# JeffOwOSun/ntm-tracker

Measured on AMD Instinct MI355X. Metric: frames/sec (whole node) VGG16+NTM(128x20) seq_len=20, higher is better.
Workload: dtype f32

## Files before the change

include/ntmtrack.h:

```cpp
#ifndef NTMTRACK_H_
#define NTMTRACK_H_

#include <stddef.h>
#include <stdint.h>

#ifdef __cplusplus
extern "C" {
#endif

#define NTK_OK               0
#define NTK_ERR_BAD_SHAPE   -1
#define NTK_ERR_BAD_PTR     -2
#define NTK_ERR_UNSUPPORTED -3
#define NTK_ERR_HIP         -4

int ntk_version(void);
const char* ntk_last_error(void);


int ntk_vgg_packed_k(int cin);
int ntk_vgg_pack_weights(const float* w_hwio, float* w_packed, int cin, int cout, void* stream);

int ntk_vgg_conv3x3_relu_f32(const float* in, const float* w_packed, const float* bias,
                             float* out, int frames, int H, int W, int cin, int cout,
// ... 4 lines not shown
                              int frames, int H, int W, int cin, int cout, int fuse_pool, int out_f32,
                              void* stream);
size_t ntk_vgg_bf16p_packed_elems(int cin, int cout);
int ntk_vgg_bf16p_supported(int H, int W, int cin, int cout, int fuse_pool);
int ntk_vgg_pack_weights_bf16p(const float* w_hwio, void* w_packed_bf16, int cin, int cout, int H, int W, void* stream);
int ntk_vgg_conv3x3_relu_bf16p(const void* in_bf16, const void* w_packed_bf16p, const float* bias, void* out,
                               int frames, int H, int W, int cin, int cout, int fuse_pool, int out_f32, void* stream);
int ntk_vgg_conv3x3_relu_f32_to_bf16(const float* in, const float* w_packed, const float* bias, void* out_bf16,
                                     int frames, int H, int W, int cin, int cout, void* stream);

size_t ntk_vgg_split3_packed_elems(int cin, int cout);
int ntk_vgg_split3_supported(int H, int W, int cin, int cout, int fuse_pool);
int ntk_vgg_pack_weights_split3(const float* w_hwio, void* w_packed, int cin, int cout, int H, int W, void* stream);
int ntk_vgg_conv3x3_relu_split3(const void* in_split, const void* w_packed, const float* bias, void* out,
                                int frames, int H, int W, int cin, int cout, int fuse_pool, int in_f32, int out_f32, void* stream);

size_t ntk_vgg_wino_packed_floats(int cin, int cout);
int ntk_vgg_wino_supported(int frames, int H, int W, int cin, int cout);
int ntk_vgg_pack_weights_wino(const float* w_hwio, float* u_packed, int cin, int cout, void* stream);
int ntk_vgg_conv3x3_relu_wino_f32(const float* in, const float* u_packed, const float* bias, float* out,
                                  int frames, int H, int W, int cin, int cout, int fuse_pool, void* stream);

size_t ntk_vgg_wino43_packed_floats(int cin, int cout);
int ntk_vgg_wino43_supported(int frames, int H, int W, int cin, int cout);
int ntk_vgg_wino43_blocked_supported(int frames, int H, int W, int cin, int cout);
int ntk_vgg_pack_weights_wino43(const float* w_hwio, float* u_packed, int cin, int cout, void* stream);
int ntk_vgg_conv3x3_relu_wino43_f32(const float* in, const float* u_packed, const float* bias, float* out,
                                    int frames, int H, int W, int cin, int cout, int fuse_pool, void* stream);
int ntk_vgg_conv3x3_relu_wino43_window_f32(const float* in, const float* u_packed, const float* bias, float* out,
                                           int frames, int H, int W, int cin, int cout, int fuse_pool,
// ... 426 lines not shown
```

ntm-tracker_amd/_lib.py:

```python
import ctypes
import os

import torch

_HERE = os.path.dirname(os.path.abspath(__file__))
LIB_PATH = os.environ.get("NTK_LIB_PATH") or os.path.join(_HERE, "libntmtrack_hip.so")

_lib = None


class NtkError(RuntimeError):
    pass


def _sig(lib):
    c_int, c_void_p, c_size_t = ctypes.c_int, ctypes.c_void_p, ctypes.c_size_t
    P = c_void_p
    sigs = {
        "ntk_version": (c_int, []),
        "ntk_last_error": (ctypes.c_char_p, []),
        "ntk_vgg_packed_k": (c_int, [c_int]),
        "ntk_vgg_pack_weights": (c_int, [P, P, c_int, c_int, P]),
        "ntk_vgg_conv3x3_relu_f32": (c_int, [P, P, P, P, c_int, c_int, c_int, c_int, c_int, c_int, P]),
        "ntk_vgg_pack_weights_bf16": (c_int, [P, P, c_int, c_int, P]),
        "ntk_vgg_conv3x3_relu_bf16": (c_int, [P, P, P, P] + [c_int] * 7 + [P]),
        "ntk_vgg_conv3x3_relu_f32_to_bf16": (c_int, [P, P, P, P] + [c_int] * 5 + [P]),
        "ntk_vgg_bf16p_packed_elems": (c_size_t, [c_int, c_int]),
        "ntk_vgg_bf16p_supported": (c_int, [c_int] * 5),
        "ntk_vgg_pack_weights_bf16p": (c_int, [P, P] + [c_int] * 4 + [P]),
        "ntk_vgg_conv3x3_relu_bf16p": (c_int, [P, P, P, P] + [c_int] * 7 + [P]),
        "ntk_vgg_split3_packed_elems": (c_size_t, [c_int, c_int]),
        "ntk_vgg_split3_supported": (c_int, [c_int] * 5),
        "ntk_vgg_pack_weights_split3": (c_int, [P, P] + [c_int] * 4 + [P]),
        "ntk_vgg_conv3x3_relu_split3": (c_int, [P, P, P, P] + [c_int] * 8 + [P]),
        "ntk_gemm_nt_f32": (c_int, [P, c_int, P, c_int, P, P, c_int, c_int, c_int, c_int, P]),
        "ntk_gemm_tn_workspace_bytes": (c_size_t, [c_int, c_int, c_int]),
        "ntk_gemm_tn_f32": (c_int, [P, c_int, P, c_int, P, c_int, c_int, c_int, c_int, c_int, c_int, P, P]),
        "ntk_ntm_padded_dims": (c_int, [c_int] * 7 + [ctypes.POINTER(c_int)] * 5),
        "ntk_ntm_seq_fwd": (c_int, [c_int] * 10 + [P] * 23 + [P]),
        "ntk_transpose_pad": (c_int, [P, c_int, P, c_int, c_int, c_int, P]),
        "ntk_ntm_seq_bwd": (c_int, [c_int] * 10 + [P, c_int, P, c_int] + [P] * 21 + [P]),
        "ntk_ntm_seq_deep_supported": (c_int, [c_int] * 9),
        "ntk_ntm_seq_plan": (c_int, [c_int] * 11 + [ctypes.POINTER(c_int)] * 4),
        "ntk_ntm_seq_deep_plan": (c_int, [c_int] * 10 + [ctypes.POINTER(c_int)] * 4),
        "ntk_ntm_seq_deep_packed_floats": (c_int, [c_int] * 5 + [ctypes.POINTER(c_size_t)] * 3),
        "ntk_ntm_seq_deep_pack": (c_int, [c_int] * 5 + [P] * 6 + [P]),
        "ntk_ntm_seq_fwd_deep": (c_int, [c_int] * 12 + [P] * 29 + [P]),
        "ntk_ntm_seq_bwd_deep": (c_int, [c_int] * 11 + [P, P, c_int] + [P] * 24 + [P]),
        "ntk_dnc_padded_dims": (c_int, [c_int] * 6 + [ctypes.POINTER(c_int)] * 8),
# ... 133 lines not shown
```

ntm-tracker_amd/csrc/conv_bf16p.hip:

```cpp
#include "conv_tiles.h"

#ifndef BF16P_ABL
#define BF16P_ABL 0
#endif

namespace {

typedef __bf16 pbf16x8 __attribute__((ext_vector_type(8)));
typedef __bf16 pbf16x4 __attribute__((ext_vector_type(4)));


struct Bf16pArgs {
    const __bf16* in; const __bf16* wq; const float* bias; void* out;
    int frames, H, W, Cin, Cout;
    int bxN, byN;
    int NQ, NS;
    int nCB;
};

typedef int pv4i __attribute__((ext_vector_type(4)));
__device__ __forceinline__ void p_dma16(pv4i rs, unsigned lds_addr, int voff, int soff) {
    unsigned keep;
    asm volatile("s_mov_b32 %0, m0\n\ts_mov_b32 m0, %1\n\ts_nop 0\n\tbuffer_load_dwordx4 %2, %3, %4 offen lds\n\ts_mov_b32 m0, %0"
                 : "=&s"(keep) : "s"(lds_addr), "v"(voff), "s"(rs), "s"(soff) : "memory");
}
__device__ __forceinline__ pv4i p_rsrc(const void* base, unsigned bytes) {
    const unsigned long long p = (unsigned long long)base;
    return pv4i{(int)(unsigned)p, (int)(unsigned)(p >> 32), (int)bytes, 0x00020000};
}

__device__ __forceinline__ pbf16x8 p_as_bf16x8(const f32x4& v) {
    union { f32x4 f; pbf16x8 b; } u;
// ... 67 lines not shown
        const int e = idx & 7;
        size_t r = idx >> 3;
        const int slot = (int)(r & 3); r >>= 2;
        const int n = (int)(r % BN); r /= BN;
        const int tap = (int)(r % 9); r /= 9;
        const int chunk = (int)(r % NC);
        const int cb = (int)(r / NC);
        const int piece = slot ^ p_sw<4>(n);
        const int c = chunk * 16 + (piece & 1) * 8 + e;
        const float v = w[((size_t)tap * Cin + c) * Cout + (size_t)cb * BN + n] * wscale;
        const _Float16 hi = (_Float16)v;
        wq[idx] = (piece & 2) ? (_Float16)(v - (float)hi) : hi;
    }
}

template <int BN, int TW, int TH, int NSUB, int KC, bool POOL, bool OUTF32, int NW = 8, bool X3 = false, bool INF32 = false>
__global__ __launch_bounds__(64 * NW) __attribute__((amdgpu_waves_per_eu(2, 2))) void conv3x3_relu_bf16p_kernel(Bf16pArgs a) {
    static_assert(!INF32 || (X3 && NW == 4), "fp32 input: split form on four waves (the eight-wave form has no registers for the staging)");
    constexpr int PNT = 2 * NW;
    constexpr bool ROWS = (TW & (TW - 1)) != 0;
    static_assert(!X3 || KC == 32, "split form: 16 real channels = one 32-channel chunk");
    static_assert(!ROWS || (!POOL && NSUB == 1 && (TW - 1 + 32 * PNT - 1) / TW + 1 <= TH - 1 && NW == 8), "runs of rows: no row pairs; TH = the patch's image rows");
    static_assert(NW == 8 || (NW == 4 && BN == 64), "four-wave workgroups take 64 columns");
    constexpr int PW = ROWS ? 32 : TW + 2, PH = TH + 2, SPX = PW * PH, NPX = NSUB * SPX;
    static_assert(!ROWS || TW + 2 <= 32, "runs of rows: the patch row pitch is 32");
    constexpr int PIXB = KC * 2, PIECES = KC / 8, PPP = 1024 / PIXB;
    constexpr int NPA = (NPX + PPP - 1) / PPP;
    constexpr int ABYTES = NPA * 1024;
    constexpr int STAPS = KC == 16 ? 9 : 3, SPC = 9 / STAPS;
    constexpr int SBYTES = STAPS * BN * PIXB, NPB = SBYTES / 1024;
    constexpr int NPAW = (NPA + NW - 1) / NW;
    constexpr int TM = BN == 128 ? 4 : 2;
    constexpr int TPS = (TW * TH) / 32;
    constexpr int K16 = KC / 16;
    static_assert(ROWS || NSUB * TW * TH == 32 * PNT, "512 (256) output pixels per workgroup");
    constexpr int TRB = POOL ? 0 : NW * TM * 32 * 144;
    constexpr int LDSB = (2 * ABYTES + 2 * SBYTES) > TRB ? (2 * ABYTES + 2 * SBYTES) : TRB;
    static_assert(LDSB + 1024 <= (NW == 8 ? 160 : 80) * 1024, "LDS");
    __shared__ __attribute__((aligned(1024))) unsigned char s_mem[LDSB];
    __shared__ int s_sbf[NSUB], s_sby[NSUB], s_sbx[NSUB];
    __shared__ __attribute__((aligned(16))) float s_bias[BN + 4];

    const int tid = threadIdx.x, lane = tid & 63;
    const int wave = __builtin_amdgcn_readfirstlane(tid >> 6);
    int cb, sp;
    conv_tile_wg(blockIdx.x, a.nCB, cb, sp);
    if (sp >= a.NS) return;
    const int H = a.H, W = a.W, Cin = a.Cin, Cout = a.Cout;
    const int rP0 = sp * (32 * PNT), rg0 = ROWS ? rP0 / TW : 0, rf0 = ROWS ? rg0 / H : 0, ry0 = ROWS ? rg0 - rf0 * H : 0;
    if (tid < BN) s_bias[tid] = a.bias[cb * BN + tid];
    if (X3 && tid == BN) s_bias[BN] = *reinterpret_cast<const float*>(a.wq + (size_t)9 * a.Cin * a.Cout);
    if constexpr (!ROWS) conv_tile_subblocks<NSUB>(s_sbf, s_sby, s_sbx, tid, sp, a.NQ, a.bxN, a.byN, TH, TW, 0, 0);
    __syncthreads();

    auto a_sw = [](int p) { return ROWS ? ((((p & 31) + 28 * (p >> 5)) >> 2) & 3) : p_sw<PIECES>(p); };
    const int f0 = ROWS ? rf0 : ((sp * NSUB) / a.bxN) / a.byN;
    const size_t in_left = (size_t)(a.frames - f0) * H * W * Cin * sizeof(__bf16);
    const unsigned in_bytes = (unsigned)(in_left < 0x7ffffff0ull ? in_left : 0x7ffffff0ull);
    const __bf16* pin = a.in + (size_t)f0 * H * W * Cin;
    unsigned aoff[NPAW];
#pragma unroll
    for (int i = 0; i < NPAW; ++i) {
        const int pa = wave + NW * i;
        const int lp = pa * PPP + lane / PIECES, slot = lane % PIECES;
        aoff[i] = 0x80000000u;
        if (pa < NPA && lp < NPX) {
            const int q = lp / SPX, rem = lp - q * SPX;
            const int py = rem / PW, px = rem - py * PW;
// ... 27 lines not shown
                const int y = s_sby[q] - 1 + py, x = s_sbx[q] - 1 + px;
                if (fq >= 0 && y >= 0 && y < H && x >= 0 && x < W)
                    foff[i] = (unsigned)(((((size_t)(fq - f0) * H + y) * W + x) * Cin) * sizeof(__bf16) + qd * 16);
            }
        }
    }
    auto f32_rsrc = [&](int chunk) {
        return __builtin_amdgcn_make_buffer_rsrc(const_cast<__bf16*>(pin + (size_t)chunk * KC), 0, (int)(in_bytes - (unsigned)chunk * PIXB), 0x00020000);
    };
    auto f32_put = [&](const f32x4& v, int dst) {
        ph16x4 h, l;
        f32x4 c;
#pragma unroll
        for (int e = 0; e < 4; ++e) c[e] = __builtin_amdgcn_fmed3f(v[e], -S3_MAX, S3_MAX);
        s3_split4(c, h, l);
        *reinterpret_cast<ph16x4*>(s_mem + dst) = h;
        *reinterpret_cast<ph16x4*>(s_mem + (dst ^ 32)) = l;
    };
    const unsigned lds0 = (unsigned)(size_t)(__attribute__((address_space(3))) void*)s_mem;
    auto dma_patch = [&](int chunk, int buf, int i0, int i1) {
        const pv4i rs = p_rsrc(pin + (size_t)chunk * KC, in_bytes - (unsigned)chunk * PIXB);
#pragma unroll
        for (int i = 0; i < NPAW; ++i) {
            if (i >= i0 && i < i1 && wave + NW * i < NPA)
                p_dma16(rs, lds0 + buf * ABYTES + (wave + NW * i) * 1024, (int)aoff[i], 0);
        }
    };
    auto dma_patch1 = [&](int chunk, int buf, auto ic) {
        constexpr int i = decltype(ic)::value;
        const pv4i rs = p_rsrc(pin + (size_t)chunk * KC, in_bytes - (unsigned)chunk * PIXB);
// ... 59 lines not shown
    for (int tm = 0; tm < TM; ++tm)
#pragma unroll
        for (int nt = 0; nt < 2; ++nt)
#pragma unroll
            for (int r = 0; r < 16; ++r) acc[tm][nt][r] = 0.f;
    const int wa0 = 2 * ABYTES + (wn * 64 + mcol) * PIXB + ((kh ^ p_sw<PIECES>(mcol)) << 4);

    if constexpr (INF32) {
        const __amdgpu_buffer_rsrc_t rs = f32_rsrc(0);
        f32x4 v[NIT];
#pragma unroll
        for (int i = 0; i < NIT; ++i) v[i] = __builtin_bit_cast(f32x4, __builtin_amdgcn_raw_buffer_load_b128(rs, (int)foff[i], 0, 0));
#pragma unroll
        for (int i = 0; i < NIT; ++i)
            if (fdst[i] >= 0) f32_put(v[i], fdst[i]);
    } else {
        dma_patch(0, 0, 0, NPAW);
    }
    dma_weights(0, 0);
    asm volatile("s_waitcnt vmcnt(0)" ::: "memory");
    __syncthreads();

    auto stage_body = [&](int chunk, auto part_c) {
        constexpr int part = decltype(part_c)::value;
        const int s = SPC * chunk + part;
        const int abuf = chunk & 1, bbuf = s & 1;
        constexpr int NDW = (NPB + NW - 1) / NW;
        constexpr int NDP = INF32 ? 0 : (NPAW + SPC - 1) / SPC;
        const bool more_w = !(BF16P_ABL & 1) && s + 1 < NSTG, more_p = !(BF16P_ABL & 1) && chunk + 1 < NC;
        auto dma_slot = [&](auto kc) {
            constexpr int k = decltype(kc)::value;
            if constexpr (k < NDW) { if (more_w) dma_weights1(s + 1, bbuf ^ 1, k); }
            else if constexpr (k < NDW + NDP && part * NDP + (k - NDW) < NPAW) {
                if (more_p) dma_patch1(chunk + 1, abuf ^ 1, ntk_ic<part * NDP + (k - NDW)>{});
            }
        };
        const int wa = wa0 + bbuf * SBYTES;
        f32x4 fst[NITS];
        if constexpr (INF32) {
            const __amdgpu_buffer_rsrc_t rs = f32_rsrc(more_p ? chunk + 1 : chunk);
#pragma unroll
            for (int j = 0; j < NITS; ++j)
                if (part * NITS + j < NIT) fst[j] = __builtin_bit_cast(f32x4, __builtin_amdgcn_raw_buffer_load_b128(rs, (int)foff[part * NITS + j], 0, 0));
        }
        if constexpr (X3) {
            f32x4 wh[2][2], wl[2], xh[TM], xl[TM];
            auto ld_w = [&](auto dc, auto kc, f32x4 (&w)[2]) {
                constexpr int dxi = decltype(dc)::value, k16 = decltype(kc)::value;
#pragma unroll
                for (int nt = 0; nt < 2; ++nt)
                    w[nt] = *reinterpret_cast<const f32x4*>(s_mem + ((wa ^ (k16 << 5)) + (dxi * BN + nt * 32) * PIXB));
// ... 9 lines not shown
                for (int tm = 0; tm < TM; ++tm)
#pragma unroll
                    for (int nt = 0; nt < 2; ++nt)
                        acc[tm][nt] = __builtin_amdgcn_mfma_f32_32x32x16_f16(p_as_f16x8(w[nt]), p_as_f16x8(x[tm]), acc[tm][nt], 0, 0, 0);
            };
            using I0 = ntk_ic<0>;
            using I1 = ntk_ic<1>;
            constexpr int NSS = STAPS * 3;
            static_assert(NDW + NDP <= NSS, "one DMA per sub-step");
            auto tapstep = [&](auto dc) {
                constexpr int dxi = decltype(dc)::value;
                if constexpr (!(BF16P_ABL & 4)) ld_w(dc, I1{}, wl);
                __builtin_amdgcn_sched_barrier(0);
                mm(wh[dxi & 1], xh);
                dma_slot(ntk_ic<3 * dxi>{});
                __builtin_amdgcn_sched_barrier(0);
                if constexpr (!(BF16P_ABL & 4)) ld_x(dc, I1{}, xl);
                __builtin_amdgcn_sched_barrier(0);
                mm(wl, xh);
                dma_slot(ntk_ic<3 * dxi + 1>{});
                __builtin_amdgcn_sched_barrier(0);
                if constexpr (dxi + 1 < STAPS && !(BF16P_ABL & 4)) {
                    ld_w(ntk_ic<dxi + 1>{}, I0{}, wh[(dxi + 1) & 1]);
                    ld_x(ntk_ic<dxi + 1>{}, I0{}, xh);
                }
                __builtin_amdgcn_sched_barrier(0);
                mm(wh[dxi & 1], xl);
                dma_slot(ntk_ic<3 * dxi + 2>{});
                __builtin_amdgcn_sched_barrier(0);
            };
            ld_w(I0{}, I0{}, wh[0]);
            ld_x(I0{}, I0{}, xh);
            if constexpr ((BF16P_ABL & 4) != 0) {
#pragma unroll
                for (int nt = 0; nt < 2; ++nt) { wh[1][nt] = wh[0][nt]; wl[nt] = wh[0][nt]; }
#pragma unroll
                for (int tm = 0; tm < TM; ++tm) xl[tm] = xh[tm];
            }
            ntk_static_for<0, STAPS>(tapstep);
            if constexpr (INF32) {
                if (more_p) {
#pragma unroll
                    for (int j = 0; j < NITS; ++j)
// ... 145 lines not shown
            for (int j = 0; j < TM * 4; ++j) {
                const int tmr = j >> 2, mr = 8 * (j & 3) + (lane >> 3), piece = lane & 7;
                const f32x4 v = *reinterpret_cast<const f32x4*>(tr + (tmr * 32 + mr) * RB + piece * 16);
                const int opx = __builtin_amdgcn_ds_bpermute(mr << 2, opix[tmr]);
                if ((BF16P_ABL & 32) ? (opx >= 0 && v[0] == 12345.f) : (opx >= 0)) {
                    const size_t op = (size_t)opx * Cout + cb * BN + wn * 64;
                    if constexpr (OUTF32) *reinterpret_cast<f32x4*>(reinterpret_cast<float*>(a.out) + op + ps * 32 + piece * 4) = v;
                    else if constexpr (X3) *reinterpret_cast<f32x4*>(reinterpret_cast<__bf16*>(a.out) + 2 * (op + ps * 32) + piece * 8) = v;
                    else *reinterpret_cast<f32x4*>(reinterpret_cast<__bf16*>(a.out) + op + piece * 8) = v;
                }
            }
        }
    }
}

template <int BN, int KC, int NW, bool X3 = false, bool INF32 = false>
int bf16p_launch(const Bf16pArgs& a0, int H, int W, int pool, int out_f32, hipStream_t st) {
    Bf16pArgs a = a0;
    if constexpr (X3 && !INF32) {
        if (W == 28) {
            if (pool || NW != 8 || H < 20) return NTK_ERR_UNSUPPORTED;
            a.bxN = 1; a.byN = 1;
            const long long NQ = (long long)a.frames * H * W, NS = (NQ + 511) / 512;
            a.NQ = 0; a.NS = (int)NS; a.nCB = a.Cout / BN;
            const unsigned grid = (unsigned)conv_tile_grid(NS, a.nCB);
            if constexpr (NW == 8) {
                if (out_f32) conv3x3_relu_bf16p_kernel<BN, 28, 21, 1, 32, false, true, 8, true><<<grid, 512, 0, st>>>(a);
                else conv3x3_relu_bf16p_kernel<BN, 28, 21, 1, 32, false, false, 8, true><<<grid, 512, 0, st>>>(a);
            }
            return NTK_OK;
        }
    }
    int shape;
    if (NW == 8) shape = (W % 32 == 0 && H % 16 == 0) ? 0 : ((W % 16 == 0 && H % 16 == 0) ? 1 : ((W % 8 == 0 && H % 8 == 0) ? 2 : 3));
    else shape = (W % 32 == 0 && H % 8 == 0) ? 0 : ((W % 16 == 0 && H % 16 == 0) ? 1 : ((W % 8 == 0 && H % 8 == 0) ? 2 : 3));
    static const int TWs[4] = {32, 16, 8, 4}, THs8[4] = {16, 16, 8, 4}, THs4[4] = {8, 16, 8, 4}, NSUB8[4] = {1, 2, 8, 32}, NSUB4[4] = {1, 1, 4, 16};
    const int TWv = TWs[shape], THv = NW == 8 ? THs8[shape] : THs4[shape], NSUBv = NW == 8 ? NSUB8[shape] : NSUB4[shape];
    a.bxN = W / TWv;
    a.byN = H / THv;
    const long long NQ = (long long)a.frames * a.bxN * a.byN;
    const long long NS = (NQ + NSUBv - 1) / NSUBv;
    a.NQ = (int)NQ; a.NS = (int)NS; a.nCB = a.Cout / BN;
    const unsigned grid = (unsigned)conv_tile_grid(NS, a.nCB);
#define BF16P_GO(TW_, TH_, NSUB_)                                                                                             \
    do {                                                                                                                      \
        if (pool) {                                                                                                           \
            if (out_f32) conv3x3_relu_bf16p_kernel<BN, TW_, TH_, NSUB_, KC, true, true, NW, X3, INF32><<<grid, 64 * NW, 0, st>>>(a);     \
            else conv3x3_relu_bf16p_kernel<BN, TW_, TH_, NSUB_, KC, true, false, NW, X3, INF32><<<grid, 64 * NW, 0, st>>>(a);            \
        } else {                                                                                                              \
            if (out_f32) conv3x3_relu_bf16p_kernel<BN, TW_, TH_, NSUB_, KC, false, true, NW, X3, INF32><<<grid, 64 * NW, 0, st>>>(a);    \
            else conv3x3_relu_bf16p_kernel<BN, TW_, TH_, NSUB_, KC, false, false, NW, X3, INF32><<<grid, 64 * NW, 0, st>>>(a);           \
        }                                                                                                                     \
    } while (0)
    if constexpr (KC == 32 && NW == 8) {
        if (shape == 0) BF16P_GO(32, 16, 1);
        else if (shape == 1) BF16P_GO(16, 16, 2);
        else if (shape == 2) BF16P_GO(8, 8, 8);
        else return NTK_ERR_UNSUPPORTED;
    } else if constexpr (KC == 32) {
        if (shape == 0) BF16P_GO(32, 8, 1);
        else if (shape == 1) BF16P_GO(16, 16, 1);
        else if (shape == 2) BF16P_GO(8, 8, 4);
        else return NTK_ERR_UNSUPPORTED;
    } else {
        if (shape == 3 && !pool && NW == 8) {
            if (out_f32) conv3x3_relu_bf16p_kernel<BN, 4, 4, 32, KC, false, true><<<grid, 512, 0, st>>>(a);
// ... 114 lines not shown
    a.in = reinterpret_cast<const __bf16*>(in_split); a.wq = reinterpret_cast<const __bf16*>(w_packed); a.bias = bias; a.out = out;
    a.frames = frames; a.H = H; a.W = W; a.Cin = 2 * cin; a.Cout = cout;
    a.bxN = a.byN = a.NQ = a.NS = a.nCB = 0;
    int rc;
    hipStream_t st = (hipStream_t)stream;
    NTK_REQUIRE(!in_f32 || nw == 4, NTK_ERR_UNSUPPORTED,
                "ntk_vgg_conv3x3_relu_split3: an fp32 input map is read by the four-wave form only (cin <= 64, cout = 64, H and W multiples of 8)");
    if (nw == 4 && in_f32) rc = bf16p_launch<64, 32, 4, true, true>(a, H, W, fuse_pool, out_f32, st);
    else if (nw == 4) rc = bf16p_launch<64, 32, 4, true>(a, H, W, fuse_pool, out_f32, st);
    else if (bn == 128) rc = bf16p_launch<128, 32, 8, true>(a, H, W, fuse_pool, out_f32, st);
    else rc = bf16p_launch<64, 32, 8, true>(a, H, W, fuse_pool, out_f32, st);
    NTK_REQUIRE(rc == NTK_OK, rc, "ntk_vgg_conv3x3_relu_split3: no instantiation for this shape");
    NTK_CHECK_LAUNCH("ntk_vgg_conv3x3_relu_split3");
    return NTK_OK;
}
```

ntm-tracker_amd/vgg.py:

```python
import math
import os
from collections import namedtuple

import torch

from . import _lib

VGG_LAYERS = [
    ("conv1_1", 3, 64, False), ("conv1_2", 64, 64, True),
    ("conv2_1", 64, 128, False), ("conv2_2", 128, 128, True),
    ("conv3_1", 128, 256, False), ("conv3_2", 256, 256, False), ("conv3_3", 256, 256, True),
    ("conv4_1", 256, 512, False), ("conv4_2", 512, 512, False), ("conv4_3", 512, 512, False),
]

def conv_flops_per_frame(h=224, w=224):
    total = 0
    for _name, cin, cout, pool in VGG_LAYERS:
        total += 2 * h * w * 9 * cin * cout
        if pool:
            h //= 2
            w //= 2
    return total


# ... 155 lines not shown
    return (s[:, :, :, :, 0].to(torch.float32) + s[:, :, :, :, 1].to(torch.float32)).reshape(F, H, W, G * 16)


def split3_supported(H, W, cin, cout, fuse_pool=False):
    return bool(_lib.lib().ntk_vgg_split3_supported(H, W, cin, cout, 1 if fuse_pool else 0))


def pack_weights_split3(w_hwio, H, W):
    kh, kw, cin, cout = w_hwio.shape
    wp = torch.empty(_lib.lib().ntk_vgg_split3_packed_elems(cin, cout), device=w_hwio.device, dtype=torch.float16)
    _lib.check(_lib.lib().ntk_vgg_pack_weights_split3(_lib.ptr(w_hwio.contiguous()), _lib.ptr(wp), cin, cout, H, W, _lib.stream()),
               "ntk_vgg_pack_weights_split3")
    return wp


def conv3x3_relu_split3(x, w_packed, bias, cin, cout, fuse_pool=False, out_f32=False, out=None):
    in_f32 = x.dtype == torch.float32
    return _conv("ntk_vgg_conv3x3_relu_split3", x, "nhwc" if in_f32 else "split", "nhwc" if out_f32 else "split", w_packed, bias,
                 cin, cout, fuse_pool, out, (1 if in_f32 else 0, 1 if out_f32 else 0),
                 "conv3x3_relu_split3: expected %s of %d channels", "an fp32 NHWC map" if in_f32 else "a split map", cin)


def pack_weights_bf16(w_hwio):
    kh, kw, cin, cout = w_hwio.shape
    wp = torch.empty((cout, 9 * cin), device=w_hwio.device, dtype=torch.bfloat16)
    _lib.check(_lib.lib().ntk_vgg_pack_weights_bf16(_lib.ptr(w_hwio.contiguous()), _lib.ptr(wp), cin, cout, _lib.stream()),
               "ntk_vgg_pack_weights_bf16")
    return wp


TrunkStep = namedtuple("TrunkStep", "layer kernel src dst pool window waves")
_STEP_FN = {"direct": "conv3x3_relu", "direct_to_bf16": "conv3x3_relu_f32_to_bf16", "wino": "conv3x3_relu_wino",
            "wino43": "conv3x3_relu_wino43", "wino43_blocked": "conv3x3_relu_wino43_blocked", "split3": "conv3x3_relu_split3",
            "bf16": "conv3x3_relu_bf16", "bf16p": "conv3x3_relu_bf16p"}


def trunk_plan(frames_shape, dtype, form, upto="conv4_3", *, layout, wino_waves, features_window, split3_upto, bf16_form):
    F, H, W = frames_shape[:3]
    names = [l[0] for l in VGG_LAYERS]
    layers = VGG_LAYERS[:names.index(upto) + 1]
    steps = []
    if dtype == "bf16":
        if upto != "conv4_3":
            raise _lib.NtkError("bf16 trunk runs to conv4_3 only")
        h, w = H, W
        for name, cin, cout, pool in layers:
            if not steps:
                kernel, src = "direct_to_bf16", "nhwc"
            else:
                patch = bf16_form == "patch" and _lib.lib().ntk_vgg_bf16p_supported(h, w, cin, cout, 1 if pool else 0)
                kernel, src = "bf16p" if patch else "bf16", "bf16"
            steps.append(TrunkStep(name, kernel, src, "nhwc" if name == upto else "bf16", pool, None, None))
# ... 21 lines not shown
                    and (src == "split" or (cin <= 64 and cout == 64))):
                kernel = "split3"
                nxt = None if last else VGG_LAYERS[li + 1]
                if nxt is not None and li + 1 <= n_split and split3_supported(oh, ow, nxt[1], nxt[2], nxt[3]):
                    dst = "split"
            else:
                kernel, dst = "wino43_blocked", "nhwc" if last else "blocked"
        elif form == "winograd" and wino43_supported(cin, cout, h, w, F):
            kernel, waves, window = "wino43", wino_waves, features_window if name == "conv4_3" else None
        elif form in ("winograd", "winograd2") and wino_supported(cin, cout, h, w, F):
            kernel = "wino"
        else:
            kernel = "direct"
        steps.append(TrunkStep(name, kernel, src, dst, pool, window, waves))
        h, w = oh, ow
    return tuple(steps)


class VGG16Conv43(object):

    def __init__(self, weights, device="cuda", chunk_frames=1024, dtype="f32", algo=None):
        self.device = torch.device(device)
        self.chunk_frames = int(chunk_frames)
        if dtype not in ("f32", "bf16"):
            raise _lib.NtkError("VGG16Conv43: dtype must be 'f32' or 'bf16'")
        if algo is None:
            algo = os.environ.get("NTK_TRUNK_ALGO", "split3")
        if algo not in ("split3", "winograd", "winograd2", "direct"):
            raise _lib.NtkError("VGG16Conv43: algo must be 'split3', 'winograd', 'winograd2' or 'direct'")
        self.dtype = dtype
        self.features_window = None
        self.split_streams = int(os.environ.get("NTK_TRUNK_SPLIT", "2" if ((dtype == "f32" and algo in ("winograd", "split3")) or dtype == "bf16") else "1"))
        self._side = []
        self.split3 = (algo == "split3" and dtype == "f32")
        self.split3_upto = os.environ.get("NTK_SPLIT3_UPTO", "conv4_3")
        self.split3_latency_frames = 12
        self._packed_split3 = {}
        self._plans = {}
        self.last_plan = None
        if self.split3:
            algo = "winograd"
        self.algo = algo
        self.wino_waves = None
        self.layout = os.environ.get("NTK_TRUNK_LAYOUT", "blocked")
        self._blocked_ws = {}
        self.packed = {}
        self._w_hwio = {}
        self._packed_bf16p = {}
        self.bf16_form = os.environ.get("NTK_BF16_FORM", "patch")
        self.packed_wino = {}
# ... 6 lines not shown
                raise _lib.NtkError("%s: weight shape %s != (3,3,%d,%d)" % (name, tuple(w.shape), cin, cout))
            if self.split3 and dtype == "f32" and cin % 16 == 0:
                self._w_hwio[name] = w
            if dtype == "bf16" and cin % 64 == 0:
                self.packed[name] = (pack_weights_bf16(w), b)
                self._w_hwio[name] = w
            else:
                self.packed[name] = (pack_weights(w), b)
                if dtype == "f32" and algo in ("winograd", "winograd2") and cin % 16 == 0:
                    self.packed_wino[name] = pack_weights_wino(w)
                    if algo == "winograd":
                        self.packed_wino43[name] = pack_weights_wino43(w)

    def _trunk_ws(self, frames, plan):
        F, H, W, _ = frames.shape
        key = (torch.cuda.current_stream(frames.device).cuda_stream, F, H, W)
        if key not in self._blocked_ws:
            if len(self._blocked_ws) >= 8:
                self._blocked_ws.clear()
            ws = (torch.empty(F * H * W * 64, device=frames.device), torch.empty(F * (H // 2) * (W // 2) * 64, device=frames.device))
            self._blocked_ws[key] = (ws, {})
        ws, views = self._blocked_ws[key]
        if plan not in views:
            if len(views) >= 8:
                views.clear()
            dsts, h, w = [], H, W
            for i, (step, (_name, _cin, cout, _pool)) in enumerate(zip(plan[:-1], VGG_LAYERS)):
                h, w = (h // 2, w // 2) if step.pool else (h, w)
                shape = _map_shape(step.dst, F, h, w, cout)
                dsts.append(ws[i & 1].view(_MAP_DTYPE[step.dst])[:math.prod(shape)].view(shape))
            views[plan] = dsts
        return views[plan]

    def split3_trunk_supported(self, frames_shape):
        F, H, W = frames_shape[:3]
        return (self.wino_waves in (None, 8) and self.features_window is None and blocked_trunk_supported(F, H, W)
                and split3_supported(H, W, 64, 64, True))

    def plan(self, frames_shape, upto="conv4_3", form=None):
        own = "split3" if self.split3 else self.algo
        if form is None:
            form = own
        elif form != own and not (form == "winograd" and self.algo == "winograd"):
            raise _lib.NtkError("VGG16Conv43: this %s trunk has no weights packed for form=%r" % (own, form))
        win = self.features_window
        key = (tuple(frames_shape[:3]), self.dtype, form, upto, self.layout, self.wino_waves, None if win is None else tuple(win),
               self.split3_upto, self.bf16_form)
        plan = self._plans.get(key)
        if plan is None:
            if len(self._plans) >= 8:
                self._plans.clear()
            plan = self._plans[key] = trunk_plan(key[0], *key[1:4], layout=key[4], wino_waves=key[5], features_window=key[6],
                                                 split3_upto=key[7], bf16_form=key[8])
        return plan

    def _step_weights(self, step, h, w, device):
        name = step.layer
        if step.kernel in ("split3", "bf16p"):
            cache, pack, key = ((self._packed_split3, pack_weights_split3, (name, h, w)) if step.kernel == "split3"
                                else (self._packed_bf16p, pack_weights_bf16p, (name, h % 8 == 0 and w % 8 == 0)))
            if key not in cache:
                cache[key] = pack(self._w_hwio[name], h, w)
                torch.cuda.current_stream(device).synchronize()
            return cache[key]
        if step.kernel in ("wino43", "wino43_blocked"):
            return self.packed_wino43[name]
        return self.packed_wino[name] if step.kernel == "wino" else self.packed[name][0]

    def forward_chunk(self, frames, upto="conv4_3", out=None, form=None):
        frames = frames.contiguous()
        F, h, w, _ = frames.shape
        plan = self.last_plan = self.plan(frames.shape, upto, form)
        launch = globals()
        dsts = self._trunk_ws(frames, plan) if len(plan) > 1 else []
        x = frames
        for i, (step, (name, cin, cout, _pool)) in enumerate(zip(plan, VGG_LAYERS)):
            if i < len(dsts):
                dst = dsts[i]
            elif out is None and step.window is not None:
                dst = torch.zeros((F, h, w, cout), device=frames.device, dtype=torch.float32)
            else:
                dst = out
            kw = {} if step.kernel == "direct_to_bf16" else {"fuse_pool": step.pool}
            if step.kernel == "wino43":
                kw.update(window=step.window, waves=step.waves)
            elif step.kernel == "wino43_blocked":
                kw["out_blocked"] = step.dst == "blocked"
            elif step.kernel in ("split3", "bf16", "bf16p"):
                kw["out_f32"] = step.dst == "nhwc"
            x = launch[_STEP_FN[step.kernel]](x, self._step_weights(step, h, w, frames.device), self.packed[name][1], cin, cout,
                                              out=dst, **kw)
            h, w = (h // 2, w // 2) if step.pool else (h, w)
        return x

    def __call__(self, frames, out=None, latency=False, form=None):
        if frames.dim() != 4 or frames.shape[3] != 3:
            raise _lib.NtkError("frames must be [F,H,W,3] NHWC")
        F, H, W, _ = frames.shape
# ... 31 lines not shown
```

Measured before the change: 13620.

## Fuse VGG conv1_1 stem into split3 conv1_2 kernel via in-kernel MFMA

```diff
diff --git a/include/ntmtrack.h b/include/ntmtrack.h
--- a/include/ntmtrack.h
+++ b/include/ntmtrack.h
@@ -42,6 +42,10 @@
 int ntk_vgg_pack_weights_split3(const float* w_hwio, void* w_packed, int cin, int cout, int H, int W, void* stream);
 int ntk_vgg_conv3x3_relu_split3(const void* in_split, const void* w_packed, const float* bias, void* out,
                                 int frames, int H, int W, int cin, int cout, int fuse_pool, int in_f32, int out_f32, void* stream);
+
+int ntk_vgg_split3_stem_supported(int H, int W, int fuse_pool);
+int ntk_vgg_conv3x3_relu_split3_stem(const float* frames_f32, const float* w1_packed, const float* bias1, const void* w2_packed,
+                                     const float* bias2, void* out, int frames, int H, int W, int fuse_pool, int out_f32, void* stream);
 
 size_t ntk_vgg_wino_packed_floats(int cin, int cout);
 int ntk_vgg_wino_supported(int frames, int H, int W, int cin, int cout);
diff --git a/ntm-tracker_amd/_lib.py b/ntm-tracker_amd/_lib.py
--- a/ntm-tracker_amd/_lib.py
+++ b/ntm-tracker_amd/_lib.py
@@ -33,6 +33,8 @@
         "ntk_vgg_split3_supported": (c_int, [c_int] * 5),
         "ntk_vgg_pack_weights_split3": (c_int, [P, P] + [c_int] * 4 + [P]),
         "ntk_vgg_conv3x3_relu_split3": (c_int, [P, P, P, P] + [c_int] * 8 + [P]),
+        "ntk_vgg_split3_stem_supported": (c_int, [c_int] * 3),
+        "ntk_vgg_conv3x3_relu_split3_stem": (c_int, [P] * 6 + [c_int] * 5 + [P]),
         "ntk_gemm_nt_f32": (c_int, [P, c_int, P, c_int, P, P, c_int, c_int, c_int, c_int, P]),
         "ntk_gemm_tn_workspace_bytes": (c_size_t, [c_int, c_int, c_int]),
         "ntk_gemm_tn_f32": (c_int, [P, c_int, P, c_int, P, c_int, c_int, c_int, c_int, c_int, c_int, P, P]),
diff --git a/ntm-tracker_amd/csrc/conv_bf16p.hip b/ntm-tracker_amd/csrc/conv_bf16p.hip
--- a/ntm-tracker_amd/csrc/conv_bf16p.hip
+++ b/ntm-tracker_amd/csrc/conv_bf16p.hip
@@ -1,4 +1,5 @@
 #include "conv_tiles.h"
+#include "conv_stem.h"
 
 #ifndef BF16P_ABL
 #define BF16P_ABL 0
@@ -16,6 +17,7 @@
     int bxN, byN;
     int NQ, NS;
     int nCB;
+    const float* stem_in = nullptr; const float* stem_w = nullptr; const float* stem_b = nullptr;
 };
 
 typedef int pv4i __attribute__((ext_vector_type(4)));
@@ -113,9 +115,10 @@
     }
 }
 
-template <int BN, int TW, int TH, int NSUB, int KC, bool POOL, bool OUTF32, int NW = 8, bool X3 = false, bool INF32 = false>
+template <int BN, int TW, int TH, int NSUB, int KC, bool POOL, bool OUTF32, int NW = 8, bool X3 = false, bool INF32 = false, bool STEM = false>
 __global__ __launch_bounds__(64 * NW) __attribute__((amdgpu_waves_per_eu(2, 2))) void conv3x3_relu_bf16p_kernel(Bf16pArgs a) {
     static_assert(!INF32 || (X3 && NW == 4), "fp32 input: split form on four waves (the eight-wave form has no registers for the staging)");
+    static_assert(!STEM || (X3 && NW == 4 && !INF32 && (TW & (TW - 1)) == 0 && TW % 2 == 0), "fused stem: split form on four waves, sub-blocks");
     constexpr int PNT = 2 * NW;
     constexpr bool ROWS = (TW & (TW - 1)) != 0;
     static_assert(!X3 || KC == 32, "split form: 16 real channels = one 32-channel chunk");
@@ -125,7 +128,7 @@
     static_assert(!ROWS || TW + 2 <= 32, "runs of rows: the patch row pitch is 32");
     constexpr int PIXB = KC * 2, PIECES = KC / 8, PPP = 1024 / PIXB;
     constexpr int NPA = (NPX + PPP - 1) / PPP;
-    constexpr int ABYTES = NPA * 1024;
+    constexpr int ABYTES = STEM ? NPX * PIXB : NPA * 1024;
     constexpr int STAPS = KC == 16 ? 9 : 3, SPC = 9 / STAPS;
     constexpr int SBYTES = STAPS * BN * PIXB, NPB = SBYTES / 1024;
     constexpr int NPAW = (NPA + NW - 1) / NW;
@@ -135,7 +138,12 @@
     static_assert(ROWS || NSUB * TW * TH == 32 * PNT, "512 (256) output pixels per workgroup");
     constexpr int TRB = POOL ? 0 : NW * TM * 32 * 144;
     constexpr int LDSB = (2 * ABYTES + 2 * SBYTES) > TRB ? (2 * ABYTES + 2 * SBYTES) : TRB;
-    static_assert(LDSB + 1024 <= (NW == 8 ? 160 : 80) * 1024, "LDS");
+    constexpr int FPW = TW + 4, FPN = STEM ? NSUB * (TH + 4) * FPW * 3 : 4;
+    constexpr int STEMB = STEM ? (FPN + 4 * 27 * 16 + 64) * 4 : 0;
+    static_assert(LDSB + STEMB + 1024 <= ((NW == 8 || (STEM && NSUB > 1)) ? 160 : 80) * 1024, "LDS");
+    __shared__ __attribute__((aligned(16))) float s_fp[FPN];
+    __shared__ __attribute__((aligned(16))) float s_w1[STEM ? 4 * 27 * 16 : 4];
+    __shared__ __attribute__((aligned(16))) float s_b1[STEM ? 64 : 4];
     __shared__ __attribute__((aligned(1024))) unsigned char s_mem[LDSB];
     __shared__ int s_sbf[NSUB], s_sby[NSUB], s_sbx[NSUB];
     __shared__ __attribute__((aligned(16))) float s_bias[BN + 4];
@@ -150,7 +158,23 @@
     if (tid < BN) s_bias[tid] = a.bias[cb * BN + tid];
     if (X3 && tid == BN) s_bias[BN] = *reinterpret_cast<const float*>(a.wq + (size_t)9 * a.Cin * a.Cout);
     if constexpr (!ROWS) conv_tile_subblocks<NSUB>(s_sbf, s_sby, s_sbx, tid, sp, a.NQ, a.bxN, a.byN, TH, TW, 0, 0);
+    if constexpr (STEM) {
+        for (int e = tid; e < 4 * 27 * 16; e += 64 * NW) {
+            const int k = (e >> 4) % 27;
+            s_w1[e] = a.stem_w[((e / (27 * 16)) * 16 + (e & 15)) * 32 + k];
+        }
+        if (tid < 64) s_b1[tid] = a.stem_b[tid];
+    }
     __syncthreads();
+    if constexpr (STEM) {
+        for (int e = tid; e < FPN; e += 64 * NW) {
+            int q, fy, fx, c, y, x;
+            stem_fp_elem(e, TW, TH, q, fy, fx, c);
+            const bool in = stem_fp_src(fy, fx, s_sby[q], s_sbx[q], H, W, y, x) && s_sbf[q] >= 0;
+            s_fp[e] = in ? a.stem_in[(((size_t)s_sbf[q] * H + y) * W + x) * 3 + c] : 0.f;
+        }
+        __syncthreads();
+    }
 
     auto a_sw = [](int p) { return ROWS ? ((((p & 31) + 28 * (p >> 5)) >> 2) & 3) : p_sw<PIECES>(p); };
     const int f0 = ROWS ? rf0 : ((sp * NSUB) / a.bxN) / a.byN;
@@ -208,6 +232,54 @@
 #pragma unroll
         for (int e = 0; e < 4; ++e) c[e] = __builtin_amdgcn_fmed3f(v[e], -S3_MAX, S3_MAX);
         s3_split4(c, h, l);
+        *reinterpret_cast<ph16x4*>(s_mem + dst) = h;
+        *reinterpret_cast<ph16x4*>(s_mem + (dst ^ 32)) = l;
+    };
+    constexpr int STILES = (NPX + 15) / 16;
+    constexpr int SNIT = STEM ? (STILES + NW - 1) / NW : 1, SNITS = (SNIT + SPC - 1) / SPC;
+    const int spi = lane & 15, sg = lane >> 4;
+    int sfo[SNIT], skof[7];
+    if constexpr (STEM) {
+#pragma unroll
+        for (int i = 0; i < SNIT; ++i) {
+            const int lp = 16 * (wave + NW * i) + spi;
+            sfo[i] = -1;
+            if (lp < NPX) {
+                int q, py, px;
+                stem_pixel(lp, TW, TH, q, py, px);
+                const bool in = s_sbf[q] >= 0 && stem_inside(py, px, s_sby[q], s_sbx[q], H, W);
+                sfo[i] = stem_fp_corner(q, py, px, TW, TH) | (in ? 0 : 0x40000000);
+            }
+        }
+#pragma unroll
+        for (int s = 0; s < 7; ++s) skof[s] = 4 * s + sg < 27 ? stem_fp_k(4 * s + sg, TW) : 0;
+    }
+    float swa[7], sxs[SNITS][7];
+    f32x4 sbv, sacc[SNITS];
+    auto stem_load = [&](int chunk, int i, int j) {
+        if (j == 0) {
+#pragma unroll
+            for (int s = 0; s < 7; ++s) swa[s] = 4 * s + sg < 27 ? s_w1[(chunk * 27 + 4 * s + sg) * 16 + spi] : 0.f;
+            sbv = *reinterpret_cast<const f32x4*>(s_b1 + chunk * 16 + 4 * sg);
+        }
+        const float* fp = s_fp + (sfo[i] < 0 ? 0 : (sfo[i] & 0xffffff));
+#pragma unroll
+        for (int s = 0; s < 7; ++s) sxs[j][s] = 4 * s + sg < 27 ? fp[skof[s]] : 0.f;
+    };
+    auto stem_mfma = [&](int j, int s) {
+        if (s == 0) sacc[j] = f32x4{0.f, 0.f, 0.f, 0.f};
+        sacc[j] = __builtin_amdgcn_mfma_f32_16x16x4f32(swa[s], sxs[j][s], sacc[j], 0, 0, 0);
+    };
+    auto stem_put = [&](int i, int j, int buf) {
+        if (sfo[i] < 0) return;
+        const int lp = 16 * (wave + NW * i) + spi;
+        const bool in = !(sfo[i] & 0x40000000);
+        f32x4 v;
+#pragma unroll
+        for (int e = 0; e < 4; ++e) v[e] = in ? __builtin_amdgcn_fmed3f(sacc[j][e] + sbv[e], 0.f, S3_MAX) : 0.f;
+        ph16x4 h, l;
+        s3_split4(v, h, l);
+        const int dst = buf * ABYTES + lp * PIXB + (((sg >> 1) ^ a_sw(lp)) << 4) + (sg & 1) * 8;
         *reinterpret_cast<ph16x4*>(s_mem + dst) = h;
         *reinterpret_cast<ph16x4*>(s_mem + (dst ^ 32)) = l;
     };
@@ -297,10 +369,19 @@
 #pragma unroll
         for (int i = 0; i < NIT; ++i)
             if (fdst[i] >= 0) f32_put(v[i], fdst[i]);
-    } else {
+    } else if constexpr (!STEM) {
         dma_patch(0, 0, 0, NPAW);
     }
     dma_weights(0, 0);
+    if constexpr (STEM) {
+#pragma unroll
+        for (int i = 0; i < SNIT; ++i) {
+            stem_load(0, i, 0);
+#pragma unroll
+            for (int s = 0; s < 7; ++s) stem_mfma(0, s);
+            stem_put(i, 0, 0);
+        }
+    }
     asm volatile("s_waitcnt vmcnt(0)" ::: "memory");
     __syncthreads();
 
@@ -309,7 +390,7 @@
         const int s = SPC * chunk + part;
         const int abuf = chunk & 1, bbuf = s & 1;
         constexpr int NDW = (NPB + NW - 1) / NW;
-        constexpr int NDP = INF32 ? 0 : (NPAW + SPC - 1) / SPC;
+        constexpr int NDP = (INF32 || STEM) ? 0 : (NPAW + SPC - 1) / SPC;
         const bool more_w = !(BF16P_ABL & 1) && s + 1 < NSTG, more_p = !(BF16P_ABL & 1) && chunk + 1 < NC;
         auto dma_slot = [&](auto kc) {
             constexpr int k = decltype(kc)::value;
@@ -318,6 +399,27 @@
                 if (more_p) dma_patch1(chunk + 1, abuf ^ 1, ntk_ic<part * NDP + (k - NDW)>{});
             }
         };
+        constexpr int SPER = (7 * SNITS + 8) / 9;
+        auto stem_slot = [&](auto kc) {
+            if constexpr (STEM) {
+                constexpr int k = decltype(kc)::value;
+                if (more_p) {
+#pragma unroll
+                    for (int u = k * SPER; u < (k + 1) * SPER && u < 7 * SNITS; ++u) {
+                        if (part * SNITS + u / 7 >= SNIT) continue;
+                        stem_mfma(u / 7, u % 7);
+                        if (u % 7 == 6) stem_put(part * SNITS + u / 7, u / 7, abuf ^ 1);
+                    }
+                }
+            }
+        };
+        if constexpr (STEM) {
+            if (more_p) {
+#pragma unroll
+                for (int j = 0; j < SNITS; ++j)
+                    if (part * SNITS + j < SNIT) stem_load(chunk + 1, part * SNITS + j, j);
+            }
+        }
         const int wa = wa0 + bbuf * SBYTES;
         f32x4 fst[NITS];
         if constexpr (INF32) {
@@ -357,11 +459,13 @@
                 __builtin_amdgcn_sched_barrier(0);
                 mm(wh[dxi & 1], xh);
                 dma_slot(ntk_ic<3 * dxi>{});
+                stem_slot(ntk_ic<3 * dxi>{});
                 __builtin_amdgcn_sched_barrier(0);
                 if constexpr (!(BF16P_ABL & 4)) ld_x(dc, I1{}, xl);
                 __builtin_amdgcn_sched_barrier(0);
                 mm(wl, xh);
                 dma_slot(ntk_ic<3 * dxi + 1>{});
+                stem_slot(ntk_ic<3 * dxi + 1>{});
                 __builtin_amdgcn_sched_barrier(0);
                 if constexpr (dxi + 1 < STAPS && !(BF16P_ABL & 4)) {
                     ld_w(ntk_ic<dxi + 1>{}, I0{}, wh[(dxi + 1) & 1]);
@@ -370,6 +474,7 @@
                 __builtin_amdgcn_sched_barrier(0);
                 mm(wh[dxi & 1], xl);
                 dma_slot(ntk_ic<3 * dxi + 2>{});
+                stem_slot(ntk_ic<3 * dxi + 2>{});
                 __builtin_amdgcn_sched_barrier(0);
             };
             ld_w(I0{}, I0{}, wh[0]);
@@ -545,7 +650,7 @@
     }
 }
 
-template <int BN, int KC, int NW, bool X3 = false, bool INF32 = false>
+template <int BN, int KC, int NW, bool X3 = false, bool INF32 = false, bool STEM = false>
 int bf16p_launch(const Bf16pArgs& a0, int H, int W, int pool, int out_f32, hipStream_t st) {
     Bf16pArgs a = a0;
     if constexpr (X3 && !INF32) {
@@ -576,11 +681,11 @@
 #define BF16P_GO(TW_, TH_, NSUB_)                                                                                             \
     do {                                                                                                                      \
         if (pool) {                                                                                                           \
-            if (out_f32) conv3x3_relu_bf16p_kernel<BN, TW_, TH_, NSUB_, KC, true, true, NW, X3, INF32><<<grid, 64 * NW, 0, st>>>(a);     \
-            else conv3x3_relu_bf16p_kernel<BN, TW_, TH_, NSUB_, KC, true, false, NW, X3, INF32><<<grid, 64 * NW, 0, st>>>(a);            \
+            if (out_f32) conv3x3_relu_bf16p_kernel<BN, TW_, TH_, NSUB_, KC, true, true, NW, X3, INF32, STEM><<<grid, 64 * NW, 0, st>>>(a);     \
+            else conv3x3_relu_bf16p_kernel<BN, TW_, TH_, NSUB_, KC, true, false, NW, X3, INF32, STEM><<<grid, 64 * NW, 0, st>>>(a);            \
         } else {                                                                                                              \
-            if (out_f32) conv3x3_relu_bf16p_kernel<BN, TW_, TH_, NSUB_, KC, false, true, NW, X3, INF32><<<grid, 64 * NW, 0, st>>>(a);    \
-            else conv3x3_relu_bf16p_kernel<BN, TW_, TH_, NSUB_, KC, false, false, NW, X3, INF32><<<grid, 64 * NW, 0, st>>>(a);           \
+            if (out_f32) conv3x3_relu_bf16p_kernel<BN, TW_, TH_, NSUB_, KC, false, true, NW, X3, INF32, STEM><<<grid, 64 * NW, 0, st>>>(a);    \
+            else conv3x3_relu_bf16p_kernel<BN, TW_, TH_, NSUB_, KC, false, false, NW, X3, INF32, STEM><<<grid, 64 * NW, 0, st>>>(a);           \
         }                                                                                                                     \
     } while (0)
     if constexpr (KC == 32 && NW == 8) {
@@ -725,3 +830,28 @@
     NTK_CHECK_LAUNCH("ntk_vgg_conv3x3_relu_split3");
     return NTK_OK;
 }
+
+extern "C" int ntk_vgg_split3_stem_supported(int H, int W, int fuse_pool) {
+    int bn = 0, nw = 0;
+    return split3_form(H, W, 64, 64, fuse_pool, &bn, &nw) && nw == 4 && (W % 8) == 0 && (H % 8) == 0;
+}
+
+extern "C" int ntk_vgg_conv3x3_relu_split3_stem(const float* frames_f32, const float* w1_packed, const float* bias1, const void* w2_packed,
+                                                const float* bias2, void* out, int frames, int H, int W, int fuse_pool, int out_f32,
+                                                void* stream) {
+    NTK_REQUIRE(frames_f32 && w1_packed && bias1 && w2_packed && bias2 && out, NTK_ERR_BAD_PTR, "ntk_vgg_conv3x3_relu_split3_stem: null pointer");
+    NTK_REQUIRE(ntk_aligned16(w2_packed) && ntk_aligned16(out) && ntk_aligned16(bias2) && (((uintptr_t)frames_f32 | (uintptr_t)w1_packed | (uintptr_t)bias1) & 3u) == 0,
+                NTK_ERR_BAD_PTR, "ntk_vgg_conv3x3_relu_split3_stem: w2_packed, bias2 and out must be 16-byte aligned, the rest 4-byte");
+    NTK_REQUIRE(frames > 0 && H > 0 && W > 0 && ntk_vgg_split3_stem_supported(H, W, fuse_pool), NTK_ERR_UNSUPPORTED,
+                "ntk_vgg_conv3x3_relu_split3_stem: frames=%d H=%d W=%d pool=%d (H, W multiples of 8)", frames, H, W, fuse_pool);
+    NTK_REQUIRE((long long)frames * H * W < (1ll << 31), NTK_ERR_UNSUPPORTED, "ntk_vgg_conv3x3_relu_split3_stem: too many pixels for 32-bit offsets");
+    Bf16pArgs a;
+    a.in = nullptr; a.wq = reinterpret_cast<const __bf16*>(w2_packed); a.bias = bias2; a.out = out;
+    a.frames = frames; a.H = H; a.W = W; a.Cin = 128; a.Cout = 64;
+    a.bxN = a.byN = a.NQ = a.NS = a.nCB = 0;
+    a.stem_in = frames_f32; a.stem_w = w1_packed; a.stem_b = bias1;
+    const int rc = bf16p_launch<64, 32, 4, true, false, true>(a, H, W, fuse_pool, out_f32, (hipStream_t)stream);
+    NTK_REQUIRE(rc == NTK_OK, rc, "ntk_vgg_conv3x3_relu_split3_stem: no instantiation for this shape");
+    NTK_CHECK_LAUNCH("ntk_vgg_conv3x3_relu_split3_stem");
+    return NTK_OK;
+}
diff --git a/ntm-tracker_amd/csrc/conv_stem.h b/ntm-tracker_amd/csrc/conv_stem.h
--- /dev/null
+++ b/ntm-tracker_amd/csrc/conv_stem.h
@@ -0,0 +1,49 @@
+#pragma once
+
+#if defined(__HIPCC__) || defined(__CUDACC__)
+#define NTK_STEM_HD __host__ __device__ __forceinline__
+#else
+#define NTK_STEM_HD static inline
+#endif
+
+NTK_STEM_HD int stem_fp_w(int tw) { return tw + 4; }
+NTK_STEM_HD int stem_fp_h(int th) { return th + 4; }
+NTK_STEM_HD int stem_fp_floats(int tw, int th, int nsub) { return nsub * stem_fp_h(th) * stem_fp_w(tw) * 3; }
+
+NTK_STEM_HD void stem_fp_elem(int e, int tw, int th, int& q, int& fy, int& fx, int& c) {
+    const int fpw = stem_fp_w(tw), fph = stem_fp_h(th);
+    c = e % 3;
+    const int p = e / 3;
+    fx = p % fpw;
+    const int r = p / fpw;
+    fy = r % fph;
+    q = r / fph;
+}
+
+NTK_STEM_HD bool stem_fp_src(int fy, int fx, int sby, int sbx, int H, int W, int& y, int& x) {
+    y = sby - 2 + fy;
+    x = sbx - 2 + fx;
+    return y >= 0 && y < H && x >= 0 && x < W;
+}
+
+NTK_STEM_HD int stem_patch_pixels(int tw, int th, int nsub) { return nsub * (th + 2) * (tw + 2); }
+NTK_STEM_HD void stem_pixel(int lp, int tw, int th, int& q, int& py, int& px) {
+    const int pw = tw + 2, ph = th + 2;
+    px = lp % pw;
+    const int r = lp / pw;
+    py = r % ph;
+    q = r / ph;
+}
+
+NTK_STEM_HD int stem_fp_corner(int q, int py, int px, int tw, int th) {
+    return ((q * stem_fp_h(th) + py) * stem_fp_w(tw) + px) * 3;
+}
+NTK_STEM_HD int stem_fp_k(int k, int tw) {
+    const int tap = k / 3, c = k - tap * 3;
+    return ((tap / 3) * stem_fp_w(tw) + tap % 3) * 3 + c;
+}
+
+NTK_STEM_HD bool stem_inside(int py, int px, int sby, int sbx, int H, int W) {
+    const int y = sby - 1 + py, x = sbx - 1 + px;
+    return y >= 0 && y < H && x >= 0 && x < W;
+}
diff --git a/ntm-tracker_amd/vgg.py b/ntm-tracker_amd/vgg.py
--- a/ntm-tracker_amd/vgg.py
+++ b/ntm-tracker_amd/vgg.py
@@ -193,7 +193,23 @@
     return wp
 
 
-def conv3x3_relu_split3(x, w_packed, bias, cin, cout, fuse_pool=False, out_f32=False, out=None):
+def split3_stem_supported(H, W, fuse_pool=False):
+    return bool(_lib.lib().ntk_vgg_split3_stem_supported(H, W, 1 if fuse_pool else 0))
+
+
+def conv3x3_relu_split3(x, w_packed, bias, cin, cout, fuse_pool=False, out_f32=False, out=None, stem=None):
+    if stem is not None:
+        if x.dim() != 4 or x.dtype != torch.float32 or x.shape[3] != 3 or (cin, cout) != (64, 64):
+            raise _lib.NtkError("conv3x3_relu_split3: the fused stem reads fp32 frames [F,H,W,3] and runs a 64 -> 64 layer")
+        F, H, W = x.shape[:3]
+        dst = "nhwc" if out_f32 else "split"
+        if out is None:
+            oh, ow = (H // 2, W // 2) if fuse_pool else (H, W)
+            out = torch.empty(_map_shape(dst, F, oh, ow, cout), device=x.device, dtype=_MAP_DTYPE[dst])
+        _lib.check(_lib.lib().ntk_vgg_conv3x3_relu_split3_stem(_lib.ptr(x), _lib.ptr(stem[0]), _lib.ptr(stem[1]), _lib.ptr(w_packed),
+                                                               _lib.ptr(bias), _lib.ptr(out), F, H, W, 1 if fuse_pool else 0,
+                                                               1 if out_f32 else 0, _lib.stream()), "ntk_vgg_conv3x3_relu_split3_stem")
+        return out
     in_f32 = x.dtype == torch.float32
     return _conv("ntk_vgg_conv3x3_relu_split3", x, "nhwc" if in_f32 else "split", "nhwc" if out_f32 else "split", w_packed, bias,
                  cin, cout, fuse_pool, out, (1 if in_f32 else 0, 1 if out_f32 else 0),
@@ -214,7 +230,8 @@
             "bf16": "conv3x3_relu_bf16", "bf16p": "conv3x3_relu_bf16p"}
 
 
-def trunk_plan(frames_shape, dtype, form, upto="conv4_3", *, layout, wino_waves, features_window, split3_upto, bf16_form):
+def trunk_plan(frames_shape, dtype, form, upto="conv4_3", *, layout, wino_waves, features_window, split3_upto, bf16_form,
+               stem="separate"):
     F, H, W = frames_shape[:3]
     names = [l[0] for l in VGG_LAYERS]
     layers = VGG_LAYERS[:names.index(upto) + 1]
@@ -266,6 +283,10 @@
             kernel = "direct"
         steps.append(TrunkStep(name, kernel, src, dst, pool, window, waves))
         h, w = oh, ow
+    if (stem == "fused" and len(steps) > 1 and steps[0].kernel == "direct" and steps[1].kernel == "split3" and steps[1].src == "nhwc"
+            and split3_stem_supported(H, W, steps[1].pool)):
+        steps[0] = steps[0]._replace(dst="stem")
+        steps[1] = steps[1]._replace(src="stem")
     return tuple(steps)
 
 
@@ -286,6 +307,9 @@
         self._side = []
         self.split3 = (algo == "split3" and dtype == "f32")
         self.split3_upto = os.environ.get("NTK_SPLIT3_UPTO", "conv4_3")
+        self.stem = os.environ.get("NTK_TRUNK_STEM", "fused")
+        if self.stem not in ("fused", "separate"):
+            raise _lib.NtkError("VGG16Conv43: NTK_TRUNK_STEM must be 'fused' or 'separate'")
         self.split3_latency_frames = 12
         self._packed_split3 = {}
         self._plans = {}
@@ -322,11 +346,13 @@
 
     def _trunk_ws(self, frames, plan):
         F, H, W, _ = frames.shape
-        key = (torch.cuda.current_stream(frames.device).cuda_stream, F, H, W)
+        fused = plan[0].dst == "stem"
+        key = (torch.cuda.current_stream(frames.device).cuda_stream, F, H, W, fused)
         if key not in self._blocked_ws:
             if len(self._blocked_ws) >= 8:
                 self._blocked_ws.clear()
-            ws = (torch.empty(F * H * W * 64, device=frames.device), torch.empty(F * (H // 2) * (W // 2) * 64, device=frames.device))
+            ws = (torch.empty(F * H * W * (32 if fused else 64), device=frames.device),
+                  torch.empty(F * (H // 2) * (W // 2) * 64, device=frames.device))
             self._blocked_ws[key] = (ws, {})
         ws, views = self._blocked_ws[key]
         if plan not in views:
@@ -335,6 +361,9 @@
             dsts, h, w = [], H, W
             for i, (step, (_name, _cin, cout, _pool)) in enumerate(zip(plan[:-1], VGG_LAYERS)):
                 h, w = (h // 2, w // 2) if step.pool else (h, w)
+                if step.dst == "stem":
+                    dsts.append(None)
+                    continue
                 shape = _map_shape(step.dst, F, h, w, cout)
                 dsts.append(ws[i & 1].view(_MAP_DTYPE[step.dst])[:math.prod(shape)].view(shape))
             views[plan] = dsts
@@ -353,13 +382,13 @@
             raise _lib.NtkError("VGG16Conv43: this %s trunk has no weights packed for form=%r" % (own, form))
         win = self.features_window
         key = (tuple(frames_shape[:3]), self.dtype, form, upto, self.layout, self.wino_waves, None if win is None else tuple(win),
-               self.split3_upto, self.bf16_form)
+               self.split3_upto, self.bf16_form, self.stem)
         plan = self._plans.get(key)
         if plan is None:
             if len(self._plans) >= 8:
                 self._plans.clear()
             plan = self._plans[key] = trunk_plan(key[0], *key[1:4], layout=key[4], wino_waves=key[5], features_window=key[6],
-                                                 split3_upto=key[7], bf16_form=key[8])
+                                                 split3_upto=key[7], bf16_form=key[8], stem=key[9])
         return plan
 
     def _step_weights(self, step, h, w, device):
@@ -389,7 +418,11 @@
                 dst = torch.zeros((F, h, w, cout), device=frames.device, dtype=torch.float32)
             else:
                 dst = out
+            if step.dst == "stem":
+                continue
             kw = {} if step.kernel == "direct_to_bf16" else {"fuse_pool": step.pool}
+            if step.src == "stem":
+                kw["stem"] = self.packed["conv1_1"]
             if step.kernel == "wino43":
                 kw.update(window=step.window, waves=step.waves)
             elif step.kernel == "wino43_blocked":
```

Result: faster. 14070, median of 6 (+3.3%).
